# HengyiWang/MorpheuS

Measured on AMD Instinct MI355X. Metric: rays/sec (fwd+bwd, 128 samples/ray), higher is better.
Workload: dtype f32 (exact 3 x bf16 operand split on the bf16 MFMA pipe, fp32 accumulate)

## Files before the change

### include/morpheus_hip.h

```cpp
#ifndef MORPHEUS_HIP_H
#define MORPHEUS_HIP_H

#include <stdint.h>

#ifdef __cplusplus
extern "C" {
#endif

#define MH_OK 0
#define MH_ERR_ARG 1
#define MH_ERR_LAUNCH 2
#define MH_ERR_OVERFLOW 3

#define MH_ABI_VERSION 9
#define MH_MAX_LEVELS 32
#define MH_TILE 32

int mh_abi_version(void);
const char *mh_status_string(int status);

int mh_grid_encode_fwd(const float *x, const float *emb, const int32_t *offsets_host,
                       const int32_t *res_host, float *out, int64_t M, int32_t L, int32_t n_levels,
                       float bound, int32_t group, void *stream);
int mh_grid_encode_bwd(const float *grad, const float *x, const float *emb,
                       const int32_t *offsets_host, const int32_t *res_host, float *grad_emb,
                       float *grad_x, int64_t M, int32_t L, int32_t n_levels, float bound, void *stream);

int64_t mh_grid_bin_workspace_ints(void);
int32_t mh_grid_bin_bricks(void);
int32_t mh_grid_bin_index_ints(void);
int mh_grid_bin_points(const float *x, int64_t M, float bound, int32_t *workspace, int32_t *perm,
                       int32_t *brick_start, void *stream);
int mh_grid_encode_bwd_binned(const float *grad, const float *x, const float *emb,
                              const int32_t *offsets_host, const int32_t *res_host, const int32_t *perm,
                              const int32_t *brick_start, float *grad_emb, int64_t *emb_acc, float *grad_x, int32_t accumulate_dx,
                              int64_t M, int32_t L, int32_t n_levels, float bound, const uint32_t *gmax_bits, void *stream);
int mh_grid_encode_fwd_binned(const float *x, const float *emb, const int32_t *offsets_host, const int32_t *res_host,
                              const int32_t *perm, const int32_t *brick_start, float *out, int64_t M, int32_t L,
                              int32_t n_levels, float bound, void *stream);
int64_t mh_grid_stage_min_points(int64_t set);

int mh_grid_general_fwd(const float *x, const float *emb, const int32_t *offsets_host, const int32_t *res_host, float *out,
                        int64_t M, int32_t L, int32_t n_levels, int32_t C, int32_t gridtype, int32_t align_corners,
                        int32_t interp, float bound, void *stream);
int mh_grid_general_bwd(const float *grad, const float *x, const float *emb, const int32_t *offsets_host,
                        const int32_t *res_host, float *grad_emb, int64_t *emb_acc, float *grad_x, int64_t M, int32_t L,
                        int32_t n_levels, int32_t C, int32_t gridtype, int32_t align_corners, int32_t interp, float bound,
                        void *stream);
int mh_grid_grad_tv(const float *x, const float *emb, const int32_t *offsets_host, const int32_t *res_host, float *grad_emb,
                    int64_t *emb_acc, float weight, int64_t M, int32_t L, int32_t C, int32_t gridtype, int32_t align_corners,
                    int32_t normalized, float bound, void *stream);
int mh_grid_grad_wd(const float *emb, const int32_t *offsets_host, float *grad_emb, float weight, int32_t L, int32_t C,
                    void *stream);

int mh_composite_fwd(const float *sigma, const float *t_starts, const float *t_ends, const float *rgb,
                     const int32_t *ray_start, const int32_t *ray_cnt, float *weights, float *opacity,
                     float *depth, float *color, int32_t N, void *stream);
int mh_composite_bwd(const float *sigma, const float *t_starts, const float *t_ends, const float *rgb,
                     const int32_t *ray_start, const int32_t *ray_cnt, const float *weights,
                     const float *g_weights, const float *g_opacity, const float *g_depth,
                     const float *g_color, float *d_sigma, float *d_rgb, int32_t N, void *stream);

int mh_generate_rays(float fx, float fy, float cx, float cy, const float *c2w_host, int32_t H, int32_t W,
                     float *rays_o, float *rays_d, void *stream);
int mh_sample_uniform(const float *rays_o, const float *rays_d, const float *jitter, int32_t N, int32_t S,
                      float bound, int32_t *ray_idx, float *t_starts, float *t_ends, float *xyz,
                      int32_t *ray_start, int32_t *ray_cnt, void *stream);

int mh_rays_sample_uniform(float fx, float fy, float cx, float cy, const float *c2w_host, int32_t H, int32_t W,
                           const int32_t *pix, const float *jitter, int32_t N, int32_t S, float bound,
                           float *rays_o, float *rays_d, int32_t *ray_idx, float *t_starts, float *t_ends,
                           float *xyz, int32_t *ray_start, int32_t *ray_cnt, void *stream);

int32_t mh_march_cap(float step, float bound);
int mh_march_slots(const float *rays_o, const float *rays_d, const float *jitter, int32_t N, float step, float bound,
                   int32_t R, const uint8_t *binary, int32_t cap, int32_t *ray_cnt, float *slot_ts, float *slot_te,
                   int32_t *overflow, void *stream);
int mh_march_pack(const int32_t *ray_start, const int32_t *ray_cnt, const float *slot_ts, const float *slot_te, int32_t N,
                  int32_t cap, int32_t *ray_idx, float *t_starts, float *t_ends, void *stream);

int mh_visibility_mask(const float *values, int32_t alpha_form, const float *t_starts, const float *t_ends,
                       const int32_t *ray_start, const int32_t *ray_cnt, int32_t N, int64_t M, float early_stop_eps,
                       const float *alpha_thre, uint8_t *keep, int32_t *kept_cnt, void *stream);
int mh_visibility_pack(const uint8_t *keep, const float *t_starts, const float *t_ends, const int32_t *ray_start,
                       const int32_t *ray_cnt, const int32_t *new_start, int32_t N, int64_t M, int64_t M_out,
                       int32_t *out_ray_idx, float *out_t_starts, float *out_t_ends, int32_t *src_index, void *stream);

int mh_fd_taps(const float *x, const float *topo, int32_t topo_dim, float eps, float bound, int64_t M, float *taps,
               float *topo6, void *stream);
int mh_fd_taps_bwd(const float *x, const float *g_taps, const float *g_topo6, int32_t topo_dim, float eps, float bound,
                   int64_t M, float *g_x, float *g_topo, void *stream);
int mh_fd_normal_fwd(const float *sdf6, float eps, int64_t M, float *normal, float *raw, void *stream);
int mh_fd_normal_bwd(const float *sdf6, const float *g_normal, const float *g_raw, float eps, int64_t M, float *g_sdf6,
                     void *stream);
int mh_sample_positions(const float *rays_o, const float *rays_d, const int32_t *ray_idx, const float *t_starts,
                        const float *t_ends, int64_t M, float *xyz, void *stream);
int mh_multicode_fwd(const float *t, const float *v0, const float *v1, const float *v2, int32_t s0, int32_t s1, int32_t s2,
                     int32_t C, int32_t F, float *out, void *stream);
int mh_multicode_bwd(const float *t, const float *g_out, float *g0, float *g1, float *g2, int32_t s0, int32_t s1, int32_t s2,
                     int32_t C, int32_t F, void *stream);
int mh_sdf_losses_fwd(const float *pred_sdf, const float *t_starts, const float *t_ends, const int32_t *ray_idx,
                      const float *rays_depth, const float *rays_mask, float trunc, int64_t M, const int32_t *n_valid,
                      float *sums, void *stream);
int mh_sdf_losses_bwd(const float *pred_sdf, const float *t_starts, const float *t_ends, const int32_t *ray_idx,
                      const float *rays_depth, const float *rays_mask, float trunc, int64_t M, const int32_t *n_valid,
                      const float *sums, const float *g_fs, const float *g_sl, float *g_pred, void *stream);
int mh_sample_positions_bwd(const float *g_xyz, const float *t_starts, const float *t_ends, const int32_t *ray_start,
                            const int32_t *ray_cnt, int32_t N, float *g_o, float *g_d, void *stream);

int64_t mh_mlp_tiles(int64_t M);
int64_t mh_warp_acts_floats(int64_t M);
int64_t mh_warp_dpre_floats(int64_t M);
int64_t mh_warp_wpack_floats(void);
int64_t mh_warp_wpackT_floats(void);
int mh_warp_fwd(const float *x, const int32_t *slot, const float *bias0_d, const float *bias0_t,
                const float *wpack_d, const float *wpack_t, const float *bias_d, const float *bias_t,
                int32_t n_bands, float *out_deform, float *out_topo, float *acts, int64_t M, void *stream);
int64_t mh_field_w3_bytes(void);
int mh_field_fwd_b3(const float *xc, const float *feat_s, const float *feat_c, const float *topo, const void *w3,
                    const float *bias, const float *beta, int32_t n_bands, int32_t with_color, float *sdf, float *sigma,
                    float *albedo, float *acts, int64_t M, void *stream);
int mh_b3_slice(const float *src, void *dst, int32_t n_layers, const int32_t *src_off_host, const int32_t *n_host,
                const int32_t *dst_off_f4_host, void *stream);
int64_t mh_warp_w3_bytes(void);
int64_t mh_warp_w3T_bytes(void);
int mh_warp_bwd_data_b3(const float *x, const float *g_deform, const float *g_topo, const void *w3T_d, const void *w3T_t,
                        int32_t n_bands, const float *acts, float *dpre, float *g_x, int64_t M, int32_t skip_dpre4, void *stream);
int32_t mh_warp_regen_dpre4(int64_t M);
int64_t mh_warp_wgrad_workspace_floats(int64_t M);
int mh_warp_wgrad_b3(const float *acts, const float *dpre, const float *g_deform, const float *g_topo, const void *w3T_d,
                     const void *w3T_t, int32_t regen_dpre4, float *workspace, float *dw_raw, float *db_raw, int64_t M, void *stream);
int64_t mh_warp_skip_zero_lines(int64_t set);
int mh_warp_fwd_b3(const float *x, const int32_t *slot, const float *bias0_d, const float *bias0_t, const void *w3_d,
                   const void *w3_t, const float *bias_d, const float *bias_t, int32_t n_bands, float *out_deform,
                   float *out_topo, float *acts, int64_t M, void *stream);
int mh_warp_bwd_data(const float *x, const float *g_deform, const float *g_topo, const float *wpackT_d,
                     const float *wpackT_t, int32_t n_bands, const float *acts, float *dpre, float *g_x,
                     int64_t M, void *stream);

int64_t mh_field_acts_floats(int64_t M);
int64_t mh_field_wpack_floats(void);
int64_t mh_field_wpackT_floats(void);
int mh_field_fwd(const float *xc, const float *feat_s, const float *feat_c, const float *topo,
                 const float *wpack, const float *bias, const float *beta, int32_t n_bands, int32_t with_color,
                 float *sdf, float *sigma, float *albedo, float *acts, int64_t M, void *stream);
int64_t mh_mlp_wgrad_workspace_floats(int32_t n_layers, const int32_t *in_feats_host,
                                      const int32_t *out_feats_host, int64_t n_tiles);
int mh_mlp_wgrad(const float *acts, const float *dpre, int64_t acts_tile_floats, int64_t dpre_tile_floats,
                 int32_t n_layers, const int32_t *act_off_host, const int32_t *dpre_off_host,
                 const int32_t *in_feats_host, const int32_t *out_feats_host, const int32_t *in_live_host,
                 const int32_t *out_live_host, float *workspace, float *dw_raw, float *db_raw, int64_t n_tiles, void *stream);
int mh_mlp_wgrad_b3(const float *acts, const float *dpre, int64_t acts_tile_floats, int64_t dpre_tile_floats,
                    int32_t n_layers, const int32_t *act_off_host, const int32_t *dpre_off_host,
                    const int32_t *in_feats_host, const int32_t *out_feats_host, const int32_t *in_live_host,
                    const int32_t *out_live_host, float *workspace, float *dw_raw, float *db_raw, int64_t n_tiles, void *stream);

int mh_weight_norm_fwd(int32_t n_layers, const float *const *v_host, const float *const *g_host, float *const *w_host,
                       const int32_t *rows_host, const int32_t *cols_host, void *stream);
int mh_weight_norm_bwd(int32_t n_layers, const float *const *v_host, const float *const *g_host,
                       const float *const *dw_host, float *const *dv_host, float *const *dg_host,
                       const int32_t *rows_host, const int32_t *cols_host, void *stream);

int64_t mh_field_bwd_fused_workspace_floats(int64_t M);
int64_t mh_field_dgeo_floats(int64_t M);
int mh_field_bwd_fused(const float *xc, const float *sdf, const float *albedo, const float *g_sdf, const float *g_sigma,
                       const float *g_albedo, const float *wpackT, const float *beta, int32_t n_bands, int32_t with_color,
                       const float *acts, float *dgeo_scratch, float *workspace, float *raw, int32_t accumulate, float *g_xc,
                       float *g_feat_s, float *g_feat_c, float *g_topo, uint32_t *gmax_bits, int64_t M, void *stream);
int64_t mh_field_w3T_bytes(void);
int mh_field_bwd_fused_b3(const float *xc, const float *sdf, const float *albedo, const float *g_sdf, const float *g_sigma,
                          const float *g_albedo, const void *w3T, const float *beta, int32_t n_bands, int32_t with_color,
                          const float *acts, float *dgeo_scratch, float *workspace, float *raw, int32_t accumulate, float *g_xc,
                          float *g_feat_s, float *g_feat_c, float *g_topo, uint32_t *gmax_bits, int64_t M, void *stream);
int64_t mh_field_bwd_pair_min_points(int64_t set);
int mh_adam_step(float *params, const float *grads, float *exp_avg, float *exp_avg_sq, int64_t n, int32_t n_segs,
                 const int64_t *seg_end_host, const float *seg_lr_host, const int64_t *seg_step_host, float beta1,
                 float beta2, float eps, void *stream);
int mh_adam_step_dev(float *params, const float *grads, float *exp_avg, float *exp_avg_sq, int64_t n, int32_t n_segs,
                     const int64_t *seg_end_host, const float *seg_lr_host, const float *seg_flag_dev, int64_t *seg_step_dev,
                     float *seg_scratch_dev, float beta1, float beta2, float eps, void *stream);

int64_t mh_adan_workspace_bytes(void);
int mh_adan_step(float *params, float *grads, float *exp_avg, float *exp_avg_sq, float *exp_avg_diff, float *neg_pre_grad,
                 int64_t n, int32_t n_segs, const int64_t *seg_end_host, const double *seg_lr_host, const int64_t *seg_step_host,
                 const int32_t *seg_flag_host, double beta1, double beta2, double beta3, double eps, double weight_decay,
                 double max_grad_norm, int32_t no_prox, void *workspace, void *stream);
int mh_adan_step_dev(float *params, float *grads, float *exp_avg, float *exp_avg_sq, float *exp_avg_diff, float *neg_pre_grad,
                     int64_t n, int32_t n_segs, const int64_t *seg_end_host, const double *seg_lr_host,
                     const int64_t *seg_step_host, const float *seg_flag_dev, int64_t *seg_seen_dev, double beta1, double beta2,
                     double beta3, double eps, double weight_decay, double max_grad_norm, int32_t no_prox, void *workspace,
                     void *stream);

int64_t mh_masked_mean_workspace_floats(void);
// ... 191 lines not shown
```

### morpheus_amd/csrc/hashgrid.hip

```cpp
#include "common.h"
#include "wave.h"
#include <stdlib.h>
#include <algorithm>
#include <atomic>
#include <cmath>

#pragma clang fp contract(off)

struct GridMeta {
    int32_t offsets[MH_MAX_LEVELS + 1];
    int32_t res[MH_MAX_LEVELS];
};

struct Corner8 {
    uint32_t row[8];
    float w[8];
};

__device__ __forceinline__ uint32_t grid_row(uint32_t cx, uint32_t cy, uint32_t cz, uint32_t res, uint32_t T,
                                             bool dense, bool pow2) {
    uint32_t idx;
    if (dense) {
        idx = cx + cy * res + cz * res * res;
        return idx;
// ... 64 lines not shown
        if (grid_locate(x, p, bound, two_bound, res, g, f)) {
            const float2 *tab = emb + meta.offsets[l];
            const uint32_t g1[3] = {min(g[0] + 1, res - 1), min(g[1] + 1, res - 1), min(g[2] + 1, res - 1)};
            uint32_t row[8];
            grid_rows8(g, g1, res, T, dense, pow2, row);
            float2 v[8];
#pragma unroll
            for (int c = 0; c < 8; c++) v[c] = tab[row[c]];
#pragma unroll
            for (int c = 0; c < 8; c++) {
                float w = ((c & 1) ? f[0] : 1.f - f[0]) * ((c & 2) ? f[1] : 1.f - f[1]) * ((c & 4) ? f[2] : 1.f - f[2]);
                r.x = fmaf(w, v[c].x, r.x);
                r.y = fmaf(w, v[c].y, r.y);
            }
        }
    }
    out[gid] = r;
}

template <int G>
__global__ __launch_bounds__(256) void grid_fwd_grouped_kernel(const float *__restrict__ x, const float2 *__restrict__ emb,
                                                               GridMeta meta, float2 *__restrict__ out, int64_t n_groups,
                                                               int L, int n_levels, float bound, float two_bound) {
    const int64_t gid = (int64_t)blockIdx.x * blockDim.x + threadIdx.x;
    const int64_t grp = gid / L;
    const int l = (int)(gid - grp * L);
    if (grp >= n_groups) return;
    if (l >= n_levels) {
#pragma unroll
        for (int i = 0; i < G; i++) out[(grp * G + i) * L + l] = make_float2(0.f, 0.f);
        return;
    }
    const uint32_t res = (uint32_t)meta.res[l];
    const uint32_t T = (uint32_t)(meta.offsets[l + 1] - meta.offsets[l]);
    const bool dense = (uint64_t)res * res * res <= (uint64_t)T;
    const bool pow2 = (T & (T - 1)) == 0;
    const float2 *tab = emb + meta.offsets[l];
    float2 v[8];
    uint32_t cg[3] = {0xffffffffu, 0xffffffffu, 0xffffffffu};
#pragma unroll
    for (int i = 0; i < G; i++) {
        const int64_t p = grp * G + i;
        uint32_t g[3];
        float f[3];
        float2 r = make_float2(0.f, 0.f);
        if (grid_locate(x, p, bound, two_bound, res, g, f)) {
            if (g[0] != cg[0] || g[1] != cg[1] || g[2] != cg[2]) {
                const uint32_t g1[3] = {min(g[0] + 1, res - 1), min(g[1] + 1, res - 1), min(g[2] + 1, res - 1)};
                uint32_t row[8];
                grid_rows8(g, g1, res, T, dense, pow2, row);
#pragma unroll
                for (int c = 0; c < 8; c++) v[c] = tab[row[c]];
                cg[0] = g[0], cg[1] = g[1], cg[2] = g[2];
            }
#pragma unroll
            for (int c = 0; c < 8; c++) {
                float w = ((c & 1) ? f[0] : 1.f - f[0]) * ((c & 2) ? f[1] : 1.f - f[1]) * ((c & 4) ? f[2] : 1.f - f[2]);
                r.x = fmaf(w, v[c].x, r.x);
                r.y = fmaf(w, v[c].y, r.y);
            }
        }
        out[p * L + l] = r;
    }
}

__device__ __forceinline__ void grid_ddx(const float2 (&v)[8], const float (&f)[3], float2 gr, float s, float (&dx)[3]) {
    float sc[8];
#pragma unroll
    for (int c = 0; c < 8; c++) sc[c] = fmaf(gr.y, v[c].y, gr.x * v[c].x);
    const float p[3][2] = {{1.f - f[0], f[0]}, {1.f - f[1], f[1]}, {1.f - f[2], f[2]}};
#pragma unroll
    for (int d = 0; d < 3; d++) {
        const int a = (d + 1) % 3, b = (d + 2) % 3;
        float acc = 0.f;
#pragma unroll
        for (int q = 0; q < 4; q++) {
            const int ba = q & 1, bb = (q >> 1) & 1;
            const int lo_c = (ba << a) | (bb << b), hi_c = lo_c | (1 << d);
            const float w = p[a][ba] * p[b][bb], diff = sc[hi_c] - sc[lo_c];
            acc = q ? fmaf(w, diff, acc) : w * diff;
        }
        dx[d] = s * acc;
    }
}

#define DPP_ADD(v, ctrl) ((v) + __int_as_float(__builtin_amdgcn_update_dpp(0, __float_as_int(v), (ctrl), 0xf, 0xf, true)))
__device__ __forceinline__ float sum16(float v) {
    v = DPP_ADD(v, 0xB1);
    v = DPP_ADD(v, 0x4E);
    v = DPP_ADD(v, 0x141);
    v = DPP_ADD(v, 0x140);
    return v;
}

template <bool NEED_DX>
__global__ __launch_bounds__(256) void grid_bwd_kernel(const float2 *__restrict__ grad, const float *__restrict__ x,
                                                       const float2 *__restrict__ emb, GridMeta meta,
                                                       float *__restrict__ grad_emb, float *__restrict__ grad_x,
                                                       int64_t M, int L, int n_levels, float bound, float two_bound) {
    const int64_t gid = (int64_t)blockIdx.x * blockDim.x + threadIdx.x;
    int64_t p = gid / L;
    const int l = (int)(gid - p * L);
    const bool live = p < M;
    if (!live) p = M - 1;
    float dx[3] = {0.f, 0.f, 0.f};
    if (live && l < n_levels) {
        const uint32_t res = (uint32_t)meta.res[l];
        const uint32_t T = (uint32_t)(meta.offsets[l + 1] - meta.offsets[l]);
        const bool dense = (uint64_t)res * res * res <= (uint64_t)T;
        const bool pow2 = (T & (T - 1)) == 0;
        uint32_t g[3];
        float f[3];
        if (grid_locate(x, p, bound, two_bound, res, g, f)) {
            const float2 gr = grad[gid];
            const uint32_t g1x = min(g[0] + 1, res - 1), g1y = min(g[1] + 1, res - 1), g1z = min(g[2] + 1, res - 1);
            uint32_t row[8];
#pragma unroll
            for (int c = 0; c < 8; c++) {
                uint32_t cx = (c & 1) ? g1x : g[0], cy = (c & 2) ? g1y : g[1], cz = (c & 4) ? g1z : g[2];
                row[c] = grid_row(cx, cy, cz, res, T, dense, pow2);
            }
            float *ge = grad_emb + (size_t)meta.offsets[l] * 2;
#pragma unroll
            for (int c = 0; c < 8; c++) {
                float w = ((c & 1) ? f[0] : 1.f - f[0]) * ((c & 2) ? f[1] : 1.f - f[1]) * ((c & 4) ? f[2] : 1.f - f[2]);
                atomicAdd(ge + (size_t)row[c] * 2 + 0, w * gr.x);
                atomicAdd(ge + (size_t)row[c] * 2 + 1, w * gr.y);
            }
            if (NEED_DX) {
                const float2 *tab = emb + meta.offsets[l];
                float2 v[8];
#pragma unroll
                for (int c = 0; c < 8; c++) v[c] = tab[row[c]];
                grid_ddx(v, f, gr, (float)res, dx);
            }
        }
    }
    if (NEED_DX) {
        float sx = sum16(dx[0]), sy = sum16(dx[1]), sz = sum16(dx[2]);
        if (live && l == 0) {
            const float inv = 1.0f / two_bound;
            grad_x[p * 3 + 0] = sx * inv;
            grad_x[p * 3 + 1] = sy * inv;
            grad_x[p * 3 + 2] = sz * inv;
        }
    }
}


#define BRK 16
#define NBRK (BRK * BRK * BRK)
#define BRK_NODES_MAX 4608

struct BrickMeta {
    int32_t n[MH_MAX_LEVELS];
    int32_t lds_off[MH_MAX_LEVELS];
};

__device__ __forceinline__ int brick_of(const float *__restrict__ x, int64_t p, float bound, float two_bound) {
    int b[3];
    const float inv = 1.0f / two_bound;
#pragma unroll
    for (int d = 0; d < 3; d++) {
        const float u = exact_div(x[p * 3 + d] + bound, two_bound, inv);
        if (!(u >= 0.0f && u <= 1.0f)) return NBRK;
        b[d] = min((int)floorf(u * (float)BRK), BRK - 1);
    }
    return (b[2] * BRK + b[1]) * BRK + b[0];
}

__global__ __launch_bounds__(256) void bin_hist_kernel(const float *__restrict__ x, int64_t M, int64_t chunk, float bound,
                                                       float two_bound, int32_t *__restrict__ block_hist) {
    __shared__ int hist[NBRK + 1];
    for (int i = threadIdx.x; i <= NBRK; i += 256) hist[i] = 0;
    __syncthreads();
    const int64_t p0 = (int64_t)blockIdx.x * chunk, p1 = min(p0 + chunk, M);
    for (int64_t p = p0 + threadIdx.x; p < p1; p += 256) atomicAdd(&hist[brick_of(x, p, bound, two_bound)], 1);
    __syncthreads();
    for (int i = threadIdx.x; i <= NBRK; i += 256) block_hist[(int64_t)blockIdx.x * (NBRK + 1) + i] = hist[i];
}

__global__ __launch_bounds__(256) void bin_colscan_kernel(int32_t *__restrict__ block_hist, int G,
                                                          int32_t *__restrict__ brick_cnt) {
    const int b = blockIdx.x * 256 + threadIdx.x;
    if (b > NBRK) return;
    int run = 0, g = 0;
    for (; g + 8 <= G; g += 8) {
        int c[8];
#pragma unroll
        for (int k = 0; k < 8; k++) c[k] = block_hist[(int64_t)(g + k) * (NBRK + 1) + b];
#pragma unroll
        for (int k = 0; k < 8; k++) {
            block_hist[(int64_t)(g + k) * (NBRK + 1) + b] = run;
            run += c[k];
        }
    }
    for (; g < G; g++) {
        const int c = block_hist[(int64_t)g * (NBRK + 1) + b];
        block_hist[(int64_t)g * (NBRK + 1) + b] = run;
        run += c;
    }
    brick_cnt[b] = run;
}

#define BRK_CHUNK_SMALL 1024
constexpr int BRK_CHUNK_LARGE = 2048;
#define BRK_CHUNK_WORD (2 * NBRK + 5)
__global__ __launch_bounds__(1024) void bin_rowscan_kernel(const int32_t *__restrict__ brick_cnt,
                                                           int32_t *__restrict__ brick_start, int chunk) {
    __shared__ int part[1024];
    __shared__ int partw[1024];
    constexpr int PER = (NBRK + 1 + 1023) / 1024;
    const int t = threadIdx.x;
    int32_t *work_start = brick_start + NBRK + 2;
    int loc[PER], locw[PER], s = 0, sw = 0;
#pragma unroll
    for (int k = 0; k < PER; k++) {
        const int i = t * PER + k;
        loc[k] = i <= NBRK ? brick_cnt[i] : 0;
        locw[k] = i < NBRK ? (loc[k] + chunk - 1) / chunk : 0;
        s += loc[k];
        sw += locw[k];
    }
    part[t] = s;
    partw[t] = sw;
    __syncthreads();
    for (int o = 1; o < 1024; o <<= 1) {
        const int v = t >= o ? part[t - o] : 0;
        const int vw = t >= o ? partw[t - o] : 0;
        __syncthreads();
        part[t] += v;
        partw[t] += vw;
        __syncthreads();
    }
    int run = part[t] - s, runw = partw[t] - sw;
#pragma unroll
    for (int k = 0; k < PER; k++) {
        const int i = t * PER + k;
        if (i <= NBRK) {
            brick_start[i] = run;
            work_start[i] = runw;
        }
        run += loc[k];
        runw += locw[k];
    }
    if (t == 1023) brick_start[NBRK + 1] = part[1023], brick_start[BRK_CHUNK_WORD] = chunk;
}

__global__ __launch_bounds__(256) void bin_scatter_kernel(const float *__restrict__ x, int64_t M, int64_t chunk, float bound,
                                                          float two_bound, const int32_t *__restrict__ block_off,
                                                          const int32_t *__restrict__ brick_start, int32_t *__restrict__ perm) {
    __shared__ int cur[NBRK + 1];
    for (int i = threadIdx.x; i <= NBRK; i += 256) cur[i] = brick_start[i] + block_off[(int64_t)blockIdx.x * (NBRK + 1) + i];
    __syncthreads();
    const int64_t p0 = (int64_t)blockIdx.x * chunk, p1 = min(p0 + chunk, M);
    for (int64_t p = p0 + threadIdx.x; p < p1; p += 256) {
        const int slot = atomicAdd(&cur[brick_of(x, p, bound, two_bound)], 1);
        perm[slot] = (int32_t)p;
    }
}

__global__ __launch_bounds__(256) void absmax_kernel(const float *__restrict__ g, int64_t n, uint32_t *__restrict__ out) {
    uint32_t m = 0;
    const int64_t stride = (int64_t)gridDim.x * blockDim.x;
    const int64_t n4 = n >> 2;
    const f32x4 *g4 = reinterpret_cast<const f32x4 *>(g);
    for (int64_t i = (int64_t)blockIdx.x * blockDim.x + threadIdx.x; i < n4; i += stride) {
        const f32x4 v = g4[i];
        m = max(max(m, __float_as_uint(fabsf(v[0]))), __float_as_uint(fabsf(v[1])));
        m = max(max(m, __float_as_uint(fabsf(v[2]))), __float_as_uint(fabsf(v[3])));
    }
    for (int64_t i = 4 * n4 + (int64_t)blockIdx.x * blockDim.x + threadIdx.x; i < n; i += stride) m = max(m, __float_as_uint(fabsf(g[i])));
    m = wave_max(m);
    if ((threadIdx.x & 63) == 0 && m) atomicMax(out, m);
}

#define FX_BITS 40
#define FX_MAGIC 6755399441055744.0
#define FX_MAGIC_BITS 0x4338000000000000ULL
#define FX_LIMIT 1099511627776.0f
__device__ __forceinline__ void fx_scales(uint32_t maxbits, float &to_fx, float &from_fx) {
    int e = (int)(maxbits >> 23) + 1;
    e = max(e, 60);
    e = min(e, 254);
    to_fx = __uint_as_float((uint32_t)(127 + FX_BITS + 127 - e) << 23);
    from_fx = __uint_as_float((uint32_t)(127 - FX_BITS - 127 + e) << 23);
}

#define BRK_THREADS 1024
constexpr int BRK_PIPE = 2;
constexpr int BRK_STAGE = 1;
constexpr int BRK_STAGE_UNROLL = 8;
constexpr int BRK_STAGE_MIN_POINTS = 1 << 20;
constexpr int BRK_STAGE_MIN = 96;

__device__ __forceinline__ int brk_div(int j, int m) { return (int)(((uint32_t)j * (uint32_t)m) >> 16); }

__device__ __forceinline__ bool brk_find_item(const int32_t *__restrict__ brick_start, int w, int *item) {
    const int32_t *work_start = brick_start + NBRK + 2;
    constexpr int PER = NBRK / BRK_THREADS;
    const int b0 = PER * (int)threadIdx.x;
    int ws[PER + 1], bs[PER + 1];
    const int chunk = brick_start[BRK_CHUNK_WORD];
#pragma unroll
    for (int k = 0; k <= PER; k++) ws[k] = work_start[b0 + k], bs[k] = brick_start[b0 + k];
    bool mine = false;
#pragma unroll
    for (int k = 0; k < PER; k++)
        if (ws[k] <= w && w < ws[k + 1]) {
            const int first = bs[k] + (w - ws[k]) * chunk;
            item[0] = b0 + k, item[1] = first, item[2] = min(first + chunk, bs[k + 1]), mine = true;
        }
    return __syncthreads_or(mine) != 0;
}

struct BrickLevel {
    uint32_t res, T, my, mz, mask, sel;
    bool dense, pow2;
    int nn, base, lo[3];
    const float2 *tab;
};

__device__ __forceinline__ BrickLevel brk_level(const GridMeta &meta, const BrickMeta &bm, const float2 *__restrict__ emb, int l,
                                                int brick) {
    BrickLevel v;
    v.res = (uint32_t)meta.res[l];
    v.T = (uint32_t)(meta.offsets[l + 1] - meta.offsets[l]);
    v.dense = (uint64_t)v.res * v.res * v.res <= (uint64_t)v.T;
    v.pow2 = (v.T & (v.T - 1)) == 0;
    v.my = v.dense ? v.res : 2654435761u, v.mz = v.dense ? v.res * v.res : 805459861u;
    v.mask = v.pow2 ? v.T - 1 : 0xffffffffu, v.sel = v.dense ? 0xffffffffu : 0u;
    v.nn = bm.n[l], v.base = bm.lds_off[l];
    const int bxyz[3] = {brick % BRK, (brick / BRK) % BRK, brick / (BRK * BRK)};
#pragma unroll
    for (int d = 0; d < 3; d++) {
        const float pos = fminf(fmaxf(fmaf((float)bxyz[d] / (float)BRK, (float)v.res, -0.5f), 0.0f), (float)(v.res - 1));
        v.lo[d] = (int)floorf(pos);
    }
    v.tab = emb + meta.offsets[l];
    return v;
}

template <int STRIDE, int OFF>
__device__ __forceinline__ void brk_stage_rows(const BrickLevel &v, int sub, long long *lds8) {
    const int n3 = v.nn * v.nn * v.nn, m = (65536 + v.nn - 1) / v.nn;
    for (int j0 = sub; j0 < n3; j0 += 64 * BRK_STAGE_UNROLL) {
        float2 r[BRK_STAGE_UNROLL];
#pragma unroll
        for (int u = 0; u < BRK_STAGE_UNROLL; u++) {
            const int j = min(j0 + 64 * u, n3 - 1);
            const int t = brk_div(j, m), jz = brk_div(t, m);
            const int jx = j - t * v.nn, jy = t - jz * v.nn;
            const uint32_t cx = min((uint32_t)(v.lo[0] + jx), v.res - 1), ym = min((uint32_t)(v.lo[1] + jy), v.res - 1) * v.my,
                           zm = min((uint32_t)(v.lo[2] + jz), v.res - 1) * v.mz;
            uint32_t row = ((cx + ym + zm) & v.sel) | ((cx ^ ym ^ zm) & v.mask & ~v.sel);
            if (__builtin_expect(!v.dense && !v.pow2, 0)) row %= v.T;
            r[u] = v.tab[row];
        }
#pragma unroll
        for (int u = 0; u < BRK_STAGE_UNROLL; u++) {
            const int j = j0 + 64 * u;
            if (j < n3) *reinterpret_cast<float2 *>(&lds8[STRIDE * (v.base + j) + OFF]) = r[u];
        }
    }
}

__global__ __launch_bounds__(BRK_THREADS, 8) void grid_fwd_brick_kernel(const float *__restrict__ x, const float2 *__restrict__ emb,
                                                                         GridMeta meta, BrickMeta bm,
                                                                         const int32_t *__restrict__ perm,
                                                                         const int32_t *__restrict__ brick_start,
                                                                         float2 *__restrict__ out, int L, int n_levels, float bound,
                                                                         float two_bound) {
    __shared__ long long val[BRK_NODES_MAX];
    __shared__ int item[3];
    const int l = threadIdx.x & 15, sub = threadIdx.x >> 4;
    constexpr int PPI = BRK_THREADS / 16;
    if (!brk_find_item(brick_start, blockIdx.x, item)) {
        const int s = (int)blockIdx.x - brick_start[NBRK + 2 + NBRK];
        const int first = brick_start[NBRK] + s * BRK_CHUNK_SMALL, stop = min(first + BRK_CHUNK_SMALL, brick_start[NBRK + 1]);
        for (int i = first + sub; i < stop; i += PPI) out[(int64_t)perm[i] * L + l] = make_float2(0.f, 0.f);
        return;
    }
    const int brick = item[0], start = item[1], end = item[2];
    const bool lev_on = l < n_levels;
    const BrickLevel lv = brk_level(meta, bm, emb, l, brick);
    if (lev_on) brk_stage_rows<1, 0>(lv, sub, val);
    __syncthreads();
    const int last = end - 1;
    int p_cur = perm[min(start + sub, last)], p_nxt = perm[min(start + sub + PPI, last)];
    float xv[3] = {x[(int64_t)p_cur * 3 + 0], x[(int64_t)p_cur * 3 + 1], x[(int64_t)p_cur * 3 + 2]};
    for (int i = start + sub; i < end; i += PPI) {
        const int p_nn = perm[min(i + 2 * PPI, last)];
        const float xn[3] = {x[(int64_t)p_nxt * 3 + 0], x[(int64_t)p_nxt * 3 + 1], x[(int64_t)p_nxt * 3 + 2]};
        float2 r = make_float2(0.f, 0.f);
        if (lev_on) {
            uint32_t g[3];
            float f[3];
            grid_locate(xv, bound, two_bound, lv.res, g, f);
            const uint32_t g1[3] = {min(g[0] + 1, lv.res - 1), min(g[1] + 1, lv.res - 1), min(g[2] + 1, lv.res - 1)};
            const int lx[2] = {(int)g[0] - lv.lo[0], (int)g1[0] - lv.lo[0]}, ly[2] = {(int)g[1] - lv.lo[1], (int)g1[1] - lv.lo[1]},
                      lz[2] = {(int)g[2] - lv.lo[2], (int)g1[2] - lv.lo[2]};
            float2 v[8];
#pragma unroll
            for (int c = 0; c < 8; c++)
                v[c] = *reinterpret_cast<const float2 *>(
                    &val[lv.base + lx[c & 1] + __mul24(lv.nn, ly[(c >> 1) & 1] + __mul24(lv.nn, lz[(c >> 2) & 1]))]);
#pragma unroll
            for (int c = 0; c < 8; c++) {
                const float w = ((c & 1) ? f[0] : 1.f - f[0]) * ((c & 2) ? f[1] : 1.f - f[1]) * ((c & 4) ? f[2] : 1.f - f[2]);
                r.x = fmaf(w, v[c].x, r.x);
                r.y = fmaf(w, v[c].y, r.y);
            }
        }
        out[(int64_t)p_cur * L + l] = r;
        p_cur = p_nxt, p_nxt = p_nn;
        xv[0] = xn[0], xv[1] = xn[1], xv[2] = xn[2];
    }
}

template <int NEED_DX, bool STAGED>
__global__ __launch_bounds__(BRK_THREADS, STAGED ? 4 : 8) void grid_bwd_brick_kernel(
    const float2 *__restrict__ grad, const float *__restrict__ x, const float2 *__restrict__ emb, GridMeta meta, BrickMeta bm,
    const int32_t *__restrict__ perm, const int32_t *__restrict__ brick_start, long long *__restrict__ emb_acc, int acc_shift,
    float *__restrict__ grad_x, int L, int n_levels, float bound, float two_bound, const uint32_t *__restrict__ gmax_bits) {
    constexpr int W = STAGED ? 3 : 2;
    __shared__ long long acc[W * BRK_NODES_MAX];
    __shared__ int item[3];
    if (!brk_find_item(brick_start, blockIdx.x, item)) return;
    const int brick = item[0], start = item[1], end = item[2];
    const bool staged = STAGED && end - start >= BRK_STAGE_MIN;
    for (int i = threadIdx.x; i < BRK_NODES_MAX; i += BRK_THREADS) acc[W * i] = 0, acc[W * i + 1] = 0;
    float to_fx, from_fx;
    fx_scales(*gmax_bits, to_fx, from_fx);
    to_fx = ldexpf(to_fx, -acc_shift);
    const float fx_lim = ldexpf(FX_LIMIT, -acc_shift);
    const int l = threadIdx.x & 15, sub = threadIdx.x >> 4;
    const bool lev_on = l < n_levels;
    const BrickLevel lv = brk_level(meta, bm, emb, l, brick);
    const uint32_t res = lv.res, T = lv.T;
    const bool dense = lv.dense, pow2 = lv.pow2;
    const int nn = lv.nn, base = lv.base;
    const int lo[3] = {lv.lo[0], lv.lo[1], lv.lo[2]};
    const float2 *tab = lv.tab;
    if (staged && lev_on) brk_stage_rows<W, 2>(lv, sub, acc);
    static_assert(MH_MAX_LEVELS >= 16, "the brick kernels run on 16-level grids (L == 16 is checked by the launchers)");
    __shared__ int flush_par[16][16];
    if (threadIdx.x < 16) {
        int *fp = flush_par[l];
        fp[0] = nn, fp[1] = (65536 + nn - 1) / nn, fp[2] = base, fp[3] = lo[0], fp[4] = lo[1], fp[5] = lo[2];
        fp[6] = (int)(res - 1), fp[7] = (int)lv.my, fp[8] = (int)lv.mz, fp[9] = (int)lv.mask, fp[10] = (int)lv.sel, fp[11] = (int)T;
        fp[12] = (int)(!dense && !pow2), fp[13] = meta.offsets[l];
    }
    __syncthreads();
    constexpr int PPI = BRK_THREADS / 16;
    const int end_r = start + ((end - start + PPI - 1) / PPI) * PPI;
    int magic_hi, magic_lo;
    asm("s_mov_b32 %0, 0x43380000" : "=s"(magic_hi));
    asm("s_mov_b32 %0, 0" : "=s"(magic_lo));
    const double magic = __longlong_as_double(((long long)magic_hi << 32) | (unsigned)magic_lo);
    const int last = end - 1;
    constexpr int PIPE = (NEED_DX && !STAGED) ? 0 : BRK_PIPE;
    int p_cur = 0, p_nxt = 0;
    float xv[3] = {0.f, 0.f, 0.f};
    float2 gr = make_float2(0.f, 0.f);
    if (PIPE == 2) {
        p_cur = perm[min(start + sub, last)];
        p_nxt = perm[min(start + sub + PPI, last)];
#pragma unroll
        for (int d = 0; d < 3; d++) xv[d] = x[(int64_t)p_cur * 3 + d];
        gr = grad[(int64_t)p_cur * L + l];
    }
    const float inv_2b = 1.0f / two_bound;
    for (int i = start + sub; i < end_r; i += PPI) {
        const bool live = i < end;
        if (PIPE == 0) p_cur = perm[min(i, last)];
        const int64_t p = p_cur;
        int p_nn = 0;
        float xn[3] = {0.f, 0.f, 0.f};
        float2 grn = make_float2(0.f, 0.f);
        if (PIPE == 2) {
            p_nn = perm[min(i + 2 * PPI, last)];
#pragma unroll
            for (int d = 0; d < 3; d++) xn[d] = x[(int64_t)p_nxt * 3 + d];
            grn = grad[(int64_t)p_nxt * L + l];
        } else {
#pragma unroll
            for (int d = 0; d < 3; d++) xv[d] = x[p * 3 + d];
            gr = grad[p * L + l];
        }
        float gx_old[3] = {0.f, 0.f, 0.f};
        if (NEED_DX == 2 && l == 0) {
#pragma unroll
            for (int d = 0; d < 3; d++) gx_old[d] = grad_x[p * 3 + d];
        }
        float dx[3] = {0.f, 0.f, 0.f};
        if (live && lev_on) {
            uint32_t g[3];
            float f[3];
            grid_locate(xv, bound, two_bound, res, g, f);
            const uint32_t g1[3] = {min(g[0] + 1, res - 1), min(g[1] + 1, res - 1), min(g[2] + 1, res - 1)};
            const int lx0 = (int)g[0] - lo[0], ly0 = (int)g[1] - lo[1], lz0 = (int)g[2] - lo[2];
            const int lx1 = (int)g1[0] - lo[0], ly1 = (int)g1[1] - lo[1], lz1 = (int)g1[2] - lo[2];
            const double gxd = (double)__builtin_amdgcn_fmed3f(gr.x * to_fx, -fx_lim, fx_lim),
                         gyd = (double)__builtin_amdgcn_fmed3f(gr.y * to_fx, -fx_lim, fx_lim);
            int slot[8];
#pragma unroll
            for (int c = 0; c < 8; c++) {
                const float w = ((c & 1) ? f[0] : 1.f - f[0]) * ((c & 2) ? f[1] : 1.f - f[1]) * ((c & 4) ? f[2] : 1.f - f[2]);
                const int li = ((c & 1) ? lx1 : lx0) + __mul24(nn, ((c & 2) ? ly1 : ly0) + __mul24(nn, (c & 4) ? lz1 : lz0));
                slot[c] = W * (base + li);
                const double wd = (double)w;
                const unsigned long long qx = (unsigned long long)__double_as_longlong(__builtin_fma(wd, gxd, magic)) - FX_MAGIC_BITS;
                const unsigned long long qy = (unsigned long long)__double_as_longlong(__builtin_fma(wd, gyd, magic)) - FX_MAGIC_BITS;
                atomicAdd(reinterpret_cast<unsigned long long *>(&acc[slot[c]]), qx);
                atomicAdd(reinterpret_cast<unsigned long long *>(&acc[slot[c] + 1]), qy);
            }
            if (NEED_DX) {
                float2 v[8];
                if (staged) {
#pragma unroll
                    for (int c = 0; c < 8; c++) v[c] = *reinterpret_cast<const float2 *>(&acc[slot[c] + 2]);
                } else {
                    uint32_t row[8];
                    grid_rows8(g, g1, res, T, dense, pow2, row);
#pragma unroll
                    for (int c = 0; c < 8; c++) v[c] = tab[row[c]];
                }
                grid_ddx(v, f, gr, (float)res, dx);
            }
        }
        if (NEED_DX) {
            const float sx = sum16(dx[0]), sy = sum16(dx[1]), sz = sum16(dx[2]);
            if (live && l == 0) {
                grad_x[p * 3 + 0] = gx_old[0] + sx * inv_2b;
                grad_x[p * 3 + 1] = gx_old[1] + sy * inv_2b;
                grad_x[p * 3 + 2] = gx_old[2] + sz * inv_2b;
            }
        }
        if (PIPE == 2) {
            p_cur = p_nxt, p_nxt = p_nn;
            xv[0] = xn[0], xv[1] = xn[1], xv[2] = xn[2], gr = grn;
        }
    }
    __syncthreads();
    {
        int total = 0;
        if (n_levels > 0) {
            const int n_last = bm.n[n_levels - 1];
            total = bm.lds_off[n_levels - 1] + n_last * n_last * n_last;
        }
        for (int j = threadIdx.x; j < total; j += BRK_THREADS) {
            const long long qx = acc[W * j], qy = acc[W * j + 1];
            if (qx == 0 && qy == 0) continue;
            int lev = 0;
#pragma unroll
            for (int k = 1; k < 16; k++) lev += (k < n_levels && j >= bm.lds_off[k]) ? 1 : 0;
            const int *fp = flush_par[lev];
            const int n = fp[0], m = fp[1], jl = j - fp[2];
            const int t = brk_div(jl, m), jz = brk_div(t, m);
            const int jx = jl - t * n, jy = t - jz * n;
            const uint32_t rmax = (uint32_t)fp[6];
            const uint32_t cx = min((uint32_t)(fp[3] + jx), rmax), ym = min((uint32_t)(fp[4] + jy), rmax) * (uint32_t)fp[7],
                           zm = min((uint32_t)(fp[5] + jz), rmax) * (uint32_t)fp[8];
            const uint32_t sel = (uint32_t)fp[10];
            uint32_t row = ((cx + ym + zm) & sel) | ((cx ^ ym ^ zm) & (uint32_t)fp[9] & ~sel);
            if (__builtin_expect(fp[12] != 0, 0)) row %= (uint32_t)fp[11];
            unsigned long long *ga = reinterpret_cast<unsigned long long *>(emb_acc + ((size_t)fp[13] + row) * 2);
            atomicAdd(ga + 0, (unsigned long long)qx);
            atomicAdd(ga + 1, (unsigned long long)qy);
        }
    }
}

__global__ void grid_acc_finalize_kernel(const long long *__restrict__ emb_acc, float *__restrict__ grad_emb, int64_t n, int acc_shift,
                                         const uint32_t *__restrict__ gmax_bits) {
    float to_fx, from_fx;
    fx_scales(*gmax_bits, to_fx, from_fx);
    const double scale = (double)from_fx * (double)(1LL << acc_shift);
    for (int64_t i = (int64_t)blockIdx.x * blockDim.x + threadIdx.x; i < n; i += (int64_t)gridDim.x * blockDim.x) {
        const long long a = emb_acc[i];
        if (a != 0) grad_emb[i] += (float)((double)a * scale);
    }
}

static int fill_meta(GridMeta &m, const int32_t *offsets_host, const int32_t *res_host, int L) {
    if (!offsets_host || !res_host || L < 1 || L > MH_MAX_LEVELS) return MH_ERR_ARG;
    for (int i = 0; i <= L; i++) m.offsets[i] = offsets_host[i];
    for (int i = 0; i < L; i++) {
        m.res[i] = res_host[i];
        if (res_host[i] < 2 || offsets_host[i + 1] <= offsets_host[i]) return MH_ERR_ARG;
    }
    return MH_OK;
}

extern "C" int mh_grid_encode_fwd(const float *x, const float *emb, const int32_t *offsets_host,
                                  const int32_t *res_host, float *out, int64_t M, int32_t L, int32_t n_levels,
                                  float bound, int32_t group, void *stream) {
    if (M == 0) return MH_OK;
    if (!x || !emb || !out || M < 0 || n_levels < 0 || n_levels > L || !(bound > 0.f) || group < 1) return MH_ERR_ARG;
    GridMeta meta;
    int st = fill_meta(meta, offsets_host, res_host, L);
    if (st) return st;
    if (group == 6 && M % 6 == 0) {
        const int64_t n_groups = M / 6;
        const int64_t gblocks = (n_groups * L + 255) / 256;
        if (gblocks > 0x7fffffffLL) return MH_ERR_ARG;
        hipLaunchKernelGGL(grid_fwd_grouped_kernel<6>, dim3((unsigned)gblocks), dim3(256), 0, mh_stream(stream), x,
                           reinterpret_cast<const float2 *>(emb), meta, reinterpret_cast<float2 *>(out), n_groups, (int)L,
                           (int)n_levels, bound, 2.0f * bound);
        MH_CHECK_LAUNCH();
        return MH_OK;
    }
    const int64_t threads = M * L;
    const int64_t blocks = (threads + 255) / 256;
    if (blocks > 0x7fffffffLL) return MH_ERR_ARG;
    hipLaunchKernelGGL(grid_fwd_kernel, dim3((unsigned)blocks), dim3(256), 0, mh_stream(stream), x,
                       reinterpret_cast<const float2 *>(emb), meta, reinterpret_cast<float2 *>(out), M, (int)L, (int)n_levels,
                       bound, 2.0f * bound);
    MH_CHECK_LAUNCH();
    return MH_OK;
}

extern "C" int mh_grid_encode_bwd(const float *grad, const float *x, const float *emb, const int32_t *offsets_host,
                                  const int32_t *res_host, float *grad_emb, float *grad_x, int64_t M, int32_t L,
                                  int32_t n_levels, float bound, void *stream) {
    if (M == 0) return MH_OK;
    if (!grad || !x || !emb || !grad_emb || M < 0 || n_levels < 0 || n_levels > L || !(bound > 0.f)) return MH_ERR_ARG;
    if (grad_x && L != 16) return MH_ERR_ARG;
    GridMeta meta;
    int st = fill_meta(meta, offsets_host, res_host, L);
    if (st) return st;
    const int64_t threads = M * L;
    const int64_t blocks = (threads + 255) / 256;
    if (blocks > 0x7fffffffLL) return MH_ERR_ARG;
    if (grad_x)
        hipLaunchKernelGGL(grid_bwd_kernel<true>, dim3((unsigned)blocks), dim3(256), 0, mh_stream(stream),
                           reinterpret_cast<const float2 *>(grad), x, reinterpret_cast<const float2 *>(emb), meta,
                           grad_emb, grad_x, M, (int)L, (int)n_levels, bound, 2.0f * bound);
    else
        hipLaunchKernelGGL(grid_bwd_kernel<false>, dim3((unsigned)blocks), dim3(256), 0, mh_stream(stream),
                           reinterpret_cast<const float2 *>(grad), x, reinterpret_cast<const float2 *>(emb), meta,
                           grad_emb, grad_x, M, (int)L, (int)n_levels, bound, 2.0f * bound);
    MH_CHECK_LAUNCH();
    return MH_OK;
}

#define BIN_BLOCKS 256
extern "C" int64_t mh_grid_bin_workspace_ints(void) { return (int64_t)BIN_BLOCKS * (NBRK + 1) + (NBRK + 1); }
extern "C" int32_t mh_grid_bin_bricks(void) { return NBRK; }
extern "C" int32_t mh_grid_bin_index_ints(void) { return 2 * NBRK + 8; }

static std::atomic<int64_t> g_stage_min_points{BRK_STAGE_MIN_POINTS};
extern "C" int64_t mh_grid_stage_min_points(int64_t set) {
    if (set >= 0) g_stage_min_points.store(set, std::memory_order_relaxed);
    return g_stage_min_points.load(std::memory_order_relaxed);
}

extern "C" int mh_grid_bin_points(const float *x, int64_t M, float bound, int32_t *workspace, int32_t *perm,
                                  int32_t *brick_start, void *stream) {
    if (M == 0) return MH_OK;
    if (!x || !workspace || !perm || !brick_start || M < 0 || M > 0x7fffffffLL || !(bound > 0.f)) return MH_ERR_ARG;
    int64_t G = (M + 1023) / 1024;
    G = G < 8 ? 8 : (G > BIN_BLOCKS ? BIN_BLOCKS : G);
    const int64_t chunk = (M + G - 1) / G;
    int32_t *block_hist = workspace, *brick_cnt = workspace + (int64_t)BIN_BLOCKS * (NBRK + 1);
    hipLaunchKernelGGL(bin_hist_kernel, dim3((unsigned)G), dim3(256), 0, mh_stream(stream), x, M, chunk, bound, 2.0f * bound,
                       block_hist);
    hipLaunchKernelGGL(bin_colscan_kernel, dim3((NBRK + 1 + 255) / 256), dim3(256), 0, mh_stream(stream), block_hist,
                       (int)G, brick_cnt);
    hipLaunchKernelGGL(bin_rowscan_kernel, dim3(1), dim3(1024), 0, mh_stream(stream), brick_cnt, brick_start,
                       M >= g_stage_min_points.load(std::memory_order_relaxed) ? BRK_CHUNK_LARGE : BRK_CHUNK_SMALL);
    hipLaunchKernelGGL(bin_scatter_kernel, dim3((unsigned)G), dim3(256), 0, mh_stream(stream), x, M, chunk, bound,
                       2.0f * bound, block_hist, brick_start, perm);
    MH_CHECK_LAUNCH();
    return MH_OK;
}

static int fill_brick_meta(BrickMeta &bm, const int32_t *res_host, int L) {
    int off = 0;
    for (int l = 0; l < L; l++) {
        const int n = (res_host[l] + BRK - 1) / BRK + 2;
        bm.n[l] = n;
        bm.lds_off[l] = off;
        off += n * n * n;
    }
    return off > BRK_NODES_MAX ? MH_ERR_ARG : MH_OK;
}

extern "C" int mh_grid_encode_fwd_binned(const float *x, const float *emb, const int32_t *offsets_host,
                                         const int32_t *res_host, const int32_t *perm, const int32_t *brick_start, float *out,
                                         int64_t M, int32_t L, int32_t n_levels, float bound, void *stream) {
    if (M == 0) return MH_OK;
    if (!x || !emb || !out || !perm || !brick_start || M < 0 || M > 0x7fffffffLL || n_levels < 0 || n_levels > L || L != 16 ||
        !(bound > 0.f))
        return MH_ERR_ARG;
    GridMeta meta;
    int st = fill_meta(meta, offsets_host, res_host, L);
    if (st) return st;
    BrickMeta bm;
    if ((st = fill_brick_meta(bm, res_host, L))) return st;
    const unsigned work_items = (unsigned)(NBRK + M / BRK_CHUNK_SMALL + 1);
    hipLaunchKernelGGL(grid_fwd_brick_kernel, dim3(work_items), dim3(BRK_THREADS), 0, mh_stream(stream), x,
                       reinterpret_cast<const float2 *>(emb), meta, bm, perm, brick_start, reinterpret_cast<float2 *>(out), (int)L,
                       (int)n_levels, bound, 2.0f * bound);
    MH_CHECK_LAUNCH();
    return MH_OK;
}

extern "C" int mh_grid_encode_bwd_binned(const float *grad, const float *x, const float *emb, const int32_t *offsets_host,
                                         const int32_t *res_host, const int32_t *perm, const int32_t *brick_start,
                                         float *grad_emb, int64_t *emb_acc, float *grad_x, int32_t accumulate_dx, int64_t M,
                                         int32_t L, int32_t n_levels, float bound, const uint32_t *gmax_bits, void *stream) {
    if (M == 0) return MH_OK;
    if (!grad || !x || !emb || !grad_emb || !emb_acc || !perm || !brick_start || M < 0 || n_levels < 0 || n_levels > L || L != 16 ||
        !(bound > 0.f))
        return MH_ERR_ARG;
    GridMeta meta;
    int st = fill_meta(meta, offsets_host, res_host, L);
    if (st) return st;
    BrickMeta bm;
    if ((st = fill_brick_meta(bm, res_host, L))) return st;
    const unsigned work_items = (unsigned)(NBRK + M / BRK_CHUNK_SMALL + 1);
    int acc_shift = 0;
    while (acc_shift < 40 && (double)M * 8.0 > std::ldexp(1.0, 62 - FX_BITS + acc_shift)) acc_shift++;
    const int64_t n_acc = (int64_t)offsets_host[L] * 2;
    if (!mh_zero_async(emb_acc, sizeof(int64_t) * (size_t)n_acc, mh_stream(stream))) return MH_ERR_LAUNCH;
    const uint32_t *gmax = gmax_bits;
    if (!gmax) {
        uint32_t *own = reinterpret_cast<uint32_t *>(const_cast<int32_t *>(brick_start)) + (2 * NBRK + 4);
        if (!mh_zero_async(own, sizeof(uint32_t), mh_stream(stream))) return MH_ERR_LAUNCH;
        hipLaunchKernelGGL(absmax_kernel, dim3(1024), dim3(256), 0, mh_stream(stream), grad, M * (int64_t)L * 2, own);
        gmax = own;
    }
#define BRK_LAUNCH(DXMODE, STG)                                                                                                \
    hipLaunchKernelGGL((grid_bwd_brick_kernel<DXMODE, STG>), dim3(work_items), dim3(BRK_THREADS), 0, mh_stream(stream),       \
                       reinterpret_cast<const float2 *>(grad), x, reinterpret_cast<const float2 *>(emb), meta, bm, perm,     \
                       brick_start, reinterpret_cast<long long *>(emb_acc), acc_shift, grad_x, (int)L, (int)n_levels, bound,          \
                       2.0f * bound, gmax)
    const bool staged = BRK_STAGE && M >= g_stage_min_points.load(std::memory_order_relaxed);
    if (grad_x && accumulate_dx) {
        if (staged) BRK_LAUNCH(2, true); else BRK_LAUNCH(2, false);
    } else if (grad_x) {
        if (!mh_zero_async(grad_x, sizeof(float) * 3 * (size_t)M, mh_stream(stream))) return MH_ERR_LAUNCH;
        if (staged) BRK_LAUNCH(1, true); else BRK_LAUNCH(1, false);
    } else {
        BRK_LAUNCH(0, false);
    }
#undef BRK_LAUNCH
    MH_CHECK_LAUNCH();
    hipLaunchKernelGGL(grid_acc_finalize_kernel, dim3((unsigned)std::min<int64_t>((n_acc + 255) / 256, 4096)), dim3(256), 0,
                       mh_stream(stream), reinterpret_cast<const long long *>(emb_acc), grad_emb, n_acc, acc_shift, gmax);
    MH_CHECK_LAUNCH();
    return MH_OK;
}
```

Baseline: 1.090 million.

## Pack staged backward LDS accumulators into bank-balanced column layout

Replaces the interleaved 3-word-per-node LDS layout in the staged brick backward kernel with a 16-column, 128-byte-stride layout. A greedy bin-packing assigns each level's x-sum, y-sum and staged-row arrays to separate columns so that per-level arrays spread across LDS banks. The aim is fewer bank conflicts on the 64-bit LDS atomics and row reads. It adds host-side layout computation, a fallback linear layout, a per-node level lookup in the flush loop, and a larger shared allocation (16*1152 words), which may lower occupancy.

```diff
diff --git a/include/morpheus_hip.h b/include/morpheus_hip.h
--- a/include/morpheus_hip.h
+++ b/include/morpheus_hip.h
@@ -39,6 +39,7 @@
                               const int32_t *perm, const int32_t *brick_start, float *out, int64_t M, int32_t L,
                               int32_t n_levels, float bound, void *stream);
 int64_t mh_grid_stage_min_points(int64_t set);
+int mh_grid_bwd_layout(const int32_t *res_host, int32_t L, int32_t *cbase, int32_t *stride, int32_t *rows);
 
 int mh_grid_general_fwd(const float *x, const float *emb, const int32_t *offsets_host, const int32_t *res_host, float *out,
                         int64_t M, int32_t L, int32_t n_levels, int32_t C, int32_t gridtype, int32_t align_corners,
diff --git a/morpheus_amd/csrc/hashgrid.hip b/morpheus_amd/csrc/hashgrid.hip
--- a/morpheus_amd/csrc/hashgrid.hip
+++ b/morpheus_amd/csrc/hashgrid.hip
@@ -240,9 +240,13 @@
 #define NBRK (BRK * BRK * BRK)
 #define BRK_NODES_MAX 4608
 
+#define BRK_ACC_ROWS 1152
+
 struct BrickMeta {
     int32_t n[MH_MAX_LEVELS];
     int32_t lds_off[MH_MAX_LEVELS];
+    int32_t cbase[3][16];
+    int32_t stride;
 };
 
 __device__ __forceinline__ int brick_of(const float *__restrict__ x, int64_t p, float bound, float two_bound) {
@@ -429,8 +433,8 @@
     return v;
 }
 
-template <int STRIDE, int OFF>
-__device__ __forceinline__ void brk_stage_rows(const BrickLevel &v, int sub, long long *lds8) {
+template <bool ZERO>
+__device__ __forceinline__ void brk_stage_rows(const BrickLevel &v, int sub, char *lds, int row0, int stride, int z0 = 0, int z1 = 0) {
     const int n3 = v.nn * v.nn * v.nn, m = (65536 + v.nn - 1) / v.nn;
     for (int j0 = sub; j0 < n3; j0 += 64 * BRK_STAGE_UNROLL) {
         float2 r[BRK_STAGE_UNROLL];
@@ -448,9 +452,17 @@
 #pragma unroll
         for (int u = 0; u < BRK_STAGE_UNROLL; u++) {
             const int j = j0 + 64 * u;
-            if (j < n3) *reinterpret_cast<float2 *>(&lds8[STRIDE * (v.base + j) + OFF]) = r[u];
-        }
-    }
+            if (j < n3) {
+                *reinterpret_cast<float2 *>(lds + row0 + j * stride) = r[u];
+                if (ZERO) *reinterpret_cast<long long *>(lds + z0 + j * stride) = 0, *reinterpret_cast<long long *>(lds + z1 + j * stride) = 0;
+            }
+        }
+    }
+}
+
+__device__ __forceinline__ void brk_zero_sums(int n3, int sub, char *lds, int stride, int z0, int z1) {
+    for (int j = sub; j < n3; j += 64)
+        *reinterpret_cast<long long *>(lds + z0 + j * stride) = 0, *reinterpret_cast<long long *>(lds + z1 + j * stride) = 0;
 }
 
 __global__ __launch_bounds__(BRK_THREADS, 8) void grid_fwd_brick_kernel(const float *__restrict__ x, const float2 *__restrict__ emb,
@@ -472,7 +484,7 @@
     const int brick = item[0], start = item[1], end = item[2];
     const bool lev_on = l < n_levels;
     const BrickLevel lv = brk_level(meta, bm, emb, l, brick);
-    if (lev_on) brk_stage_rows<1, 0>(lv, sub, val);
+    if (lev_on) brk_stage_rows<false>(lv, sub, reinterpret_cast<char *>(val), 8 * lv.base, 8);
     __syncthreads();
     const int last = end - 1;
     int p_cur = perm[min(start + sub, last)], p_nxt = perm[min(start + sub + PPI, last)];
@@ -511,13 +523,15 @@
     const float2 *__restrict__ grad, const float *__restrict__ x, const float2 *__restrict__ emb, GridMeta meta, BrickMeta bm,
     const int32_t *__restrict__ perm, const int32_t *__restrict__ brick_start, long long *__restrict__ emb_acc, int acc_shift,
     float *__restrict__ grad_x, int L, int n_levels, float bound, float two_bound, const uint32_t *__restrict__ gmax_bits) {
-    constexpr int W = STAGED ? 3 : 2;
-    __shared__ long long acc[W * BRK_NODES_MAX];
+    constexpr int ACC_WORDS = STAGED ? 16 * BRK_ACC_ROWS : 2 * BRK_NODES_MAX;
+    __shared__ long long acc[ACC_WORDS];
+    char *accb = reinterpret_cast<char *>(acc);
     __shared__ int item[3];
     if (!brk_find_item(brick_start, blockIdx.x, item)) return;
     const int brick = item[0], start = item[1], end = item[2];
     const bool staged = STAGED && end - start >= BRK_STAGE_MIN;
-    for (int i = threadIdx.x; i < BRK_NODES_MAX; i += BRK_THREADS) acc[W * i] = 0, acc[W * i + 1] = 0;
+    if (!STAGED)
+        for (int i = threadIdx.x; i < BRK_NODES_MAX; i += BRK_THREADS) acc[2 * i] = 0, acc[2 * i + 1] = 0;
     float to_fx, from_fx;
     fx_scales(*gmax_bits, to_fx, from_fx);
     to_fx = ldexpf(to_fx, -acc_shift);
@@ -530,14 +544,20 @@
     const int nn = lv.nn, base = lv.base;
     const int lo[3] = {lv.lo[0], lv.lo[1], lv.lo[2]};
     const float2 *tab = lv.tab;
-    if (staged && lev_on) brk_stage_rows<W, 2>(lv, sub, acc);
+    const int stride = STAGED ? bm.stride : 16;
+    const int cb0 = STAGED ? bm.cbase[0][l] : 16 * base, cb1 = STAGED ? bm.cbase[1][l] : cb0 + 8, cb2 = STAGED ? bm.cbase[2][l] : 0;
+    const int d1 = cb1 - cb0, d2 = cb2 - cb0;
+    if (STAGED && lev_on) {
+        if (staged) brk_stage_rows<true>(lv, sub, accb, cb2, stride, cb0, cb1);
+        else brk_zero_sums(nn * nn * nn, sub, accb, stride, cb0, cb1);
+    }
     static_assert(MH_MAX_LEVELS >= 16, "the brick kernels run on 16-level grids (L == 16 is checked by the launchers)");
     __shared__ int flush_par[16][16];
     if (threadIdx.x < 16) {
         int *fp = flush_par[l];
         fp[0] = nn, fp[1] = (65536 + nn - 1) / nn, fp[2] = base, fp[3] = lo[0], fp[4] = lo[1], fp[5] = lo[2];
         fp[6] = (int)(res - 1), fp[7] = (int)lv.my, fp[8] = (int)lv.mz, fp[9] = (int)lv.mask, fp[10] = (int)lv.sel, fp[11] = (int)T;
-        fp[12] = (int)(!dense && !pow2), fp[13] = meta.offsets[l];
+        fp[12] = (int)(!dense && !pow2), fp[13] = meta.offsets[l], fp[14] = cb0, fp[15] = cb1;
     }
     __syncthreads();
     constexpr int PPI = BRK_THREADS / 16;
@@ -596,18 +616,18 @@
             for (int c = 0; c < 8; c++) {
                 const float w = ((c & 1) ? f[0] : 1.f - f[0]) * ((c & 2) ? f[1] : 1.f - f[1]) * ((c & 4) ? f[2] : 1.f - f[2]);
                 const int li = ((c & 1) ? lx1 : lx0) + __mul24(nn, ((c & 2) ? ly1 : ly0) + __mul24(nn, (c & 4) ? lz1 : lz0));
-                slot[c] = W * (base + li);
+                slot[c] = cb0 + __mul24(li, stride);
                 const double wd = (double)w;
                 const unsigned long long qx = (unsigned long long)__double_as_longlong(__builtin_fma(wd, gxd, magic)) - FX_MAGIC_BITS;
                 const unsigned long long qy = (unsigned long long)__double_as_longlong(__builtin_fma(wd, gyd, magic)) - FX_MAGIC_BITS;
-                atomicAdd(reinterpret_cast<unsigned long long *>(&acc[slot[c]]), qx);
-                atomicAdd(reinterpret_cast<unsigned long long *>(&acc[slot[c] + 1]), qy);
+                atomicAdd(reinterpret_cast<unsigned long long *>(accb + slot[c]), qx);
+                atomicAdd(reinterpret_cast<unsigned long long *>(accb + slot[c] + d1), qy);
             }
             if (NEED_DX) {
                 float2 v[8];
                 if (staged) {
 #pragma unroll
-                    for (int c = 0; c < 8; c++) v[c] = *reinterpret_cast<const float2 *>(&acc[slot[c] + 2]);
+                    for (int c = 0; c < 8; c++) v[c] = *reinterpret_cast<const float2 *>(accb + slot[c] + d2);
                 } else {
                     uint32_t row[8];
                     grid_rows8(g, g1, res, T, dense, pow2, row);
@@ -638,11 +658,19 @@
             total = bm.lds_off[n_levels - 1] + n_last * n_last * n_last;
         }
         for (int j = threadIdx.x; j < total; j += BRK_THREADS) {
-            const long long qx = acc[W * j], qy = acc[W * j + 1];
+            int lev = 0;
+            if (STAGED) {
+#pragma unroll
+                for (int k = 1; k < 16; k++) lev += (k < n_levels && j >= bm.lds_off[k]) ? 1 : 0;
+            }
+            const int a0 = STAGED ? flush_par[lev][14] + (j - flush_par[lev][2]) * stride : 16 * j;
+            const int a1 = STAGED ? flush_par[lev][15] + (j - flush_par[lev][2]) * stride : 16 * j + 8;
+            const long long qx = *reinterpret_cast<const long long *>(accb + a0), qy = *reinterpret_cast<const long long *>(accb + a1);
             if (qx == 0 && qy == 0) continue;
-            int lev = 0;
-#pragma unroll
-            for (int k = 1; k < 16; k++) lev += (k < n_levels && j >= bm.lds_off[k]) ? 1 : 0;
+            if (!STAGED) {
+#pragma unroll
+                for (int k = 1; k < 16; k++) lev += (k < n_levels && j >= bm.lds_off[k]) ? 1 : 0;
+            }
             const int *fp = flush_par[lev];
             const int n = fp[0], m = fp[1], jl = j - fp[2];
             const int t = brk_div(jl, m), jz = brk_div(t, m);
@@ -765,6 +793,7 @@
 }
 
 static int fill_brick_meta(BrickMeta &bm, const int32_t *res_host, int L) {
+    bm = BrickMeta{};
     int off = 0;
     for (int l = 0; l < L; l++) {
         const int n = (res_host[l] + BRK - 1) / BRK + 2;
@@ -773,6 +802,62 @@
         off += n * n * n;
     }
     return off > BRK_NODES_MAX ? MH_ERR_ARG : MH_OK;
+}
+
+static int brick_layout_linear(BrickMeta &bm) {
+    for (int k = 0; k < 3; k++)
+        for (int l = 0; l < 16; l++) bm.cbase[k][l] = 8 * (3 * bm.lds_off[l] + k);
+    bm.stride = 24;
+    return (24 * (bm.lds_off[15] + bm.n[15] * bm.n[15] * bm.n[15]) + 127) / 128;
+}
+
+static int brick_layout(BrickMeta &bm) {
+    int sz[16], col[3][16], h[16] = {}, order[48];
+    bool used[3][16] = {};
+    for (int l = 0; l < 16; l++) sz[l] = bm.n[l] * bm.n[l] * bm.n[l];
+    for (int i = 0; i < 48; i++) order[i] = i;
+    std::stable_sort(order, order + 48, [&](int a, int b) { return sz[a % 16] > sz[b % 16]; });
+    for (int i = 0; i < 48; i++) {
+        const int k = order[i] / 16, l = order[i] % 16;
+        int best = -1;
+        for (int c = 0; c < 16; c++)
+            if (!used[k][c] && (best < 0 || h[c] < h[best])) best = c;
+        used[k][best] = true, col[k][l] = best, h[best] += sz[l];
+    }
+    for (bool moved = true; moved;) {
+        moved = false;
+        for (int k = 0; k < 3; k++)
+            for (int a = 0; a < 16; a++)
+                for (int b = a + 1; b < 16; b++) {
+                    const int ca = col[k][a], cb = col[k][b], d = sz[a] - sz[b];
+                    if (std::max(h[ca] - d, h[cb] + d) < std::max(h[ca], h[cb]))
+                        h[ca] -= d, h[cb] += d, col[k][a] = cb, col[k][b] = ca, moved = true;
+                }
+    }
+    const int rows = *std::max_element(h, h + 16);
+    if (rows > BRK_ACC_ROWS) return brick_layout_linear(bm);
+    int top[16] = {};
+    for (int k = 0; k < 3; k++)
+        for (int l = 0; l < 16; l++) {
+            const int c = col[k][l];
+            bm.cbase[k][l] = 128 * top[c] + 8 * c;
+            top[c] += sz[l];
+        }
+    bm.stride = 128;
+    return rows;
+}
+
+extern "C" int mh_grid_bwd_layout(const int32_t *res_host, int32_t L, int32_t *cbase, int32_t *stride, int32_t *rows) {
+    if (!res_host || !cbase || !stride || !rows || L != 16) return MH_ERR_ARG;
+    for (int l = 0; l < L; l++)
+        if (res_host[l] < 2) return MH_ERR_ARG;
+    BrickMeta bm;
+    if (int st = fill_brick_meta(bm, res_host, L)) return st;
+    *rows = brick_layout(bm);
+    *stride = bm.stride;
+    for (int k = 0; k < 3; k++)
+        for (int l = 0; l < 16; l++) cbase[16 * k + l] = bm.cbase[k][l];
+    return MH_OK;
 }
 
 extern "C" int mh_grid_encode_fwd_binned(const float *x, const float *emb, const int32_t *offsets_host,
@@ -808,6 +893,8 @@
     if (st) return st;
     BrickMeta bm;
     if ((st = fill_brick_meta(bm, res_host, L))) return st;
+    const bool staged = BRK_STAGE && grad_x && M >= g_stage_min_points.load(std::memory_order_relaxed);
+    if (staged) brick_layout(bm);
     const unsigned work_items = (unsigned)(NBRK + M / BRK_CHUNK_SMALL + 1);
     int acc_shift = 0;
     while (acc_shift < 40 && (double)M * 8.0 > std::ldexp(1.0, 62 - FX_BITS + acc_shift)) acc_shift++;
@@ -825,7 +912,6 @@
                        reinterpret_cast<const float2 *>(grad), x, reinterpret_cast<const float2 *>(emb), meta, bm, perm,     \
                        brick_start, reinterpret_cast<long long *>(emb_acc), acc_shift, grad_x, (int)L, (int)n_levels, bound,          \
                        2.0f * bound, gmax)
-    const bool staged = BRK_STAGE && M >= g_stage_min_points.load(std::memory_order_relaxed);
     if (grad_x && accumulate_dx) {
         if (staged) BRK_LAUNCH(2, true); else BRK_LAUNCH(2, false);
     } else if (grad_x) {
```

Result: faster. 1.106 million (median of 6 runs) (+1.5%).
